# flashlight/wav2letter

Hardware: AMD Instinct MI355X
Metric: utterances/sec (higher is better)
Workload: dtype f32

## Files before the change

### include/fl_compat/flashlight.h

```cpp
#pragma once
#include <stdint.h>
#include <cstdio>
#include <initializer_list>

#include <functional>
#include <memory>
#include <stdexcept>
#include <string>
#include <type_traits>
#include <unordered_map>
#include <utility>
#include <vector>

#define FL_COMPAT_API __attribute__((visibility("default")))

namespace af {
typedef long long dim_t;

class FL_COMPAT_API dim4 {
 public:
  dim_t dims[4];
  dim4(dim_t d0 = 1, dim_t d1 = 1, dim_t d2 = 1, dim_t d3 = 1) : dims{d0, d1, d2, d3} {}
  dim_t elements() const { return dims[0] * dims[1] * dims[2] * dims[3]; }
  dim_t ndims() const {
// ... 386 lines not shown

 private:
  std::shared_ptr<fl::Sequential> net_;
  std::shared_ptr<void> state_;
  void* h_ = nullptr;
  int slots_ = 0, maxChunk_ = 0, maxOut_ = 0, nFeat_ = 0, nLabel_ = 0;
  bool mixed_ = false;
};

class FL_COMPAT_API SequenceCriterion : public fl::Container {
 public:
  std::vector<Variable> forward(const std::vector<Variable>& inputs) override = 0;
  virtual af::array viterbiPath(const af::array& input, const af::array& inputSize = af::array()) = 0;
  virtual af::array viterbiPathWithTarget(const af::array& input, const af::array& target,
                                          const af::array& inputSizes = af::array(), const af::array& targetSizes = af::array()) = 0;
  std::string prettyString() const override = 0;
};

struct FlatView { float* ptr; size_t floats; };
FL_COMPAT_API FlatView flatParameters(const std::shared_ptr<fl::Module>& network);
FL_COMPAT_API FlatView flatGradients(const std::shared_ptr<fl::Module>& network);
FL_COMPAT_API void setMixedPrecision(const std::shared_ptr<fl::Module>& network, bool on);
FL_COMPAT_API void setMixedPrecisionConvolutions(const std::shared_ptr<fl::Module>& network, bool on);
FL_COMPAT_API uint32_t networkStep(const std::shared_ptr<fl::Module>& network);
FL_COMPAT_API void setNetworkStep(const std::shared_ptr<fl::Module>& network, uint32_t step);

class NGramLM;
class Lexicon;

struct BeamSearchOptions {
  int beamSize = 64;
  int beamSizeToken = 64;
  float beamThreshold = 1.0f / 0.0f;
  bool logAdd = false;
  int normalize = -1;
  int nbest = 1;
  int maxLen = 0;
  const NGramLM* lm = nullptr;
  float lmWeight = 0.f;
  af::array classScore;
  float eosScore = 0.f;
  const Lexicon* lexicon = nullptr;
  float wordScore = 0.f;
  int maxWords = 0;
  bool wide = false;
};
// ... 84 lines not shown
```

### include/w2l_hip.h

```cpp
#ifndef W2L_HIP_H_
#define W2L_HIP_H_

#include <stddef.h>
#include <stdint.h>

#ifdef __cplusplus
extern "C" {
#endif

typedef void* w2l_stream_t;

typedef enum {
  W2L_OK = 0,
  W2L_EINVAL = 1,
  W2L_EHIP = 2,
  W2L_EUNSUPPORTED = 3
} w2l_status;

typedef enum {
  W2L_SCALE_NONE = 0,
  W2L_SCALE_INPUT_SZ = 1,
  W2L_SCALE_INPUT_SZ_SQRT = 2,
  W2L_SCALE_TARGET_SZ = 3,
  W2L_SCALE_TARGET_SZ_SQRT = 4
// ... 359 lines not shown
int w2l_trainer_param_info(void* h, int i, char* name, int nameCap, size_t* numel, size_t* offset);
int w2l_trainer_init_params(void* h, float* h_params, uint64_t seed);
int w2l_trainer_import_param(void* h, int i, const float* h_ref, float* h_params);
int w2l_trainer_export_param(void* h, int i, const float* h_arena, float* h_ref);
int w2l_trainer_plan(void* h, int B, int T, int L, size_t* arenaFloats, size_t* critWsBytes, int* Tout);
int w2l_trainer_bind(void* h, float* params, float* grads, float* momentum, float* arena, void* critWs);
int w2l_trainer_forward(void* h, const float* x, int train, const float** emission, void* stream);
int w2l_trainer_forward_backward(void* h, const float* x, const int* target, float** lossDev,
                                 void* stream);
int w2l_trainer_backward(void* handle, const float* dEmission, void* stream);
int w2l_trainer_update(void* h, float lr, float lrcrit, float momentum, float maxGradNorm,
                       float totalBatch, int clampCrit, void* stream);
int w2l_trainer_skipped_updates(void* h, uint64_t* count, void* stream);
int w2l_trainer_set_optimizer(void* h, int netKind, int critKind);
int w2l_trainer_set_input_sizes(void* h, const float* inputSizesDev);
int w2l_trainer_bind_state2(void* h, float* state2);
int w2l_trainer_viterbi(void* h, const float* emission, int* path, void* stream);
int w2l_trainer_evaluate(void* h, const float* x, const int* target, float** lossDev, int** pathDev, void* stream);
size_t w2l_trainer_eval_bytes(void* h);
int w2l_trainer_bind_eval(void* h, void* mem, size_t bytes);
int w2l_trainer_set_step(void* h, uint32_t step);
int w2l_trainer_set_mixed_precision(void* h, int on);
int w2l_trainer_set_mixed_precision_convs(void* h, int on);
int w2l_trainer_set_dropout(void* h, double pDropout, double pLayerDrop);
int w2l_trainer_grad_norm(void* h, double* norm, void* stream);
int w2l_trainer_set_linseg(void* h, uint32_t updates);
int w2l_trainer_set_grad_buckets(void* h, int n, const size_t* offsets);
int w2l_trainer_wait_bucket(void* h, int k, void* stream);
int w2l_profile_enable(int on);
int w2l_profile_report(int* launches, double* totalMs, double* totalFlops);
int w2l_profile_report_kind(int kind, int* launches, double* totalMs, double* totalWork);
int w2l_profile_launches(int kind, int maxRows, double* ms, double* work, int* dims);
int w2l_arch_check(const char* archText, int nFeat, int nLabel, int* numLayers);
int w2l_flags_check(const char* flagsText, int* numFlags);

int w2l_stream_create(const char* archText, int nFeat, int nLabel, int slots, int maxChunk, void** session);
int w2l_stream_create_for_trainer(void* trainer, int slots, int maxChunk, void** session);
void w2l_stream_destroy(void* session);
int w2l_stream_query(const char* archText, int nFeat, int nLabel, int slots, int maxChunk, int* maxOut, size_t* stateBytes);
int w2l_stream_max_out(void* session);
size_t w2l_stream_state_bytes(void* session);
size_t w2l_stream_param_floats(void* session);
int w2l_stream_num_time_layers(void* session);
int w2l_stream_bind(void* session, const float* params, void* state, size_t stateBytes);
int w2l_stream_counts(void* session, const int* n, const int* start, const int* finish, int* nOut);
int w2l_stream_slot_state(void* session, int slot, int* active, int* carry, int carryCap);
// ... 50 lines not shown
```

### wav2letter_amd/csrc/gemm.hip

```cpp
#include <atomic>
#include <cstdlib>
#include <map>
#include <mutex>
#include <utility>

#include "gemm.hpp"
#include "gemm_glds.hpp"
#include "gemm_t160.hpp"
#include "gemm_bf16.hpp"
#include "gemm_bf16g.hpp"

namespace w2l {

GemmProf& gemm_prof() {
  static GemmProf p;
  return p;
}

float* sk_scratch(hipStream_t s, size_t bytes) {
  static std::mutex mu;
  static std::map<std::pair<int, hipStream_t>, std::pair<float*, size_t>> cache;
  int dev = 0;
  if (hipGetDevice(&dev) != hipSuccess) return nullptr;
  std::lock_guard<std::mutex> lk(mu);
  auto& e = cache[{dev, s}];
  if (e.second < bytes) {
    if (e.first) (void)hipFree(e.first);
    e.first = nullptr;
    e.second = 0;
    void* p = nullptr;
    if (hipMalloc(&p, bytes) != hipSuccess) return nullptr;
    e.first = (float*)p;
    e.second = bytes;
  }
  return e.first;
}

static bool glds_enabled() {
  const char* e = tune_env("W2L_GEMM_GLDS");
  return !(e && e[0] == '0');
}

static inline bool glds_ok(const float* p, int ld, int extent) {
  return (((uintptr_t)p) & 15) == 0 && ld % 4 == 0 && extent % 4 == 0 && extent >= 4;
}
static inline bool glds_ok_relaxed(const float* p, int extent) {
  return (((uintptr_t)p) & 3) == 0 && extent >= 4;
}

unsigned* sk_counters(hipStream_t s) {
  static std::mutex mu;
  static std::map<std::pair<int, hipStream_t>, unsigned*> cache;
  int dev = 0;
  if (hipGetDevice(&dev) != hipSuccess) return nullptr;
  std::lock_guard<std::mutex> lk(mu);
  unsigned*& e = cache[{dev, s}];
  if (!e) {
    void* p = nullptr;
    if (hipMalloc(&p, 1024 * sizeof(unsigned)) != hipSuccess) return nullptr;
    if (hipMemset(p, 0, 1024 * sizeof(unsigned)) != hipSuccess) { (void)hipFree(p); return nullptr; }
    e = (unsigned*)p;
  }
  return e;
}

template <class AOp>
static int dispatch_b(const AOp& a, const float* B, int ldb, int b_kcontig, const GemmOut& o, int epi, hipStream_t s) {
  if (b_kcontig) {
    int v = pick_vec(B, ldb, o.K);
    if (v == 4) return launch128(a, PlainOp<true, 4>{B, ldb, o.N, o.K}, o, epi, s);
    if (v == 2) return launch128(a, PlainOp<true, 2>{B, ldb, o.N, o.K}, o, epi, s);
    return launch128(a, PlainOp<true, 1>{B, ldb, o.N, o.K}, o, epi, s);
  }
  int v = pick_vec(B, ldb, o.N);
  if (v == 4) return launch128(a, PlainOp<false, 4>{B, ldb, o.N, o.K}, o, epi, s);
  if (v == 2) return launch128(a, PlainOp<false, 2>{B, ldb, o.N, o.K}, o, epi, s);
  return launch128(a, PlainOp<false, 1>{B, ldb, o.N, o.K}, o, epi, s);
}

static std::atomic<int> g_matmul_bf16{0};

static int gemm_bf16(const float* A, int lda, int a_kcontig, const float* B, int ldb, int b_kcontig, const GemmOut& o, int epi,
                     hipStream_t s) {
  const bool va = pick_vec(A, lda, a_kcontig ? o.K : o.M) == 4, vb = pick_vec(B, ldb, b_kcontig ? o.K : o.N) == 4;
  if (a_kcontig) {
    const BfOp<true> a{A, lda, o.M, o.K, va};
// ... 248 lines not shown
```

### wav2letter_amd/csrc/host/fl_compat.cpp

```cpp
#include <dlfcn.h>
#include <time.h>

#include <algorithm>
#include <cmath>
#include <cstring>
#include <sstream>
#include <unordered_map>
#include <unordered_set>

#include "../../../include/fl_compat/flashlight.h"
#include "../../../include/fl_compat/lexicon.h"
#include "../../../include/fl_compat/lm.h"
#include "w2l_host.hpp"

namespace {

hipStream_t g_stream = nullptr;
bool g_streamUser = false;

hipStream_t S() {
  if (!g_stream) w2l::hipCheck(hipStreamCreateWithFlags(&g_stream, hipStreamNonBlocking), "fl_compat stream");
  return g_stream;
}

// ... 1030 lines not shown
hipEvent_t arenaBucketEvent(void* net, size_t k) { return ((pkg::speech::PlannedNet*)net)->bucketEvents_.at(k); }
void arenaInstallBuckets(void* net, std::vector<size_t> offs) { ((pkg::speech::PlannedNet*)net)->installBuckets(std::move(offs)); }
}
namespace pkg {
namespace speech {

namespace {
PlannedNet* plannedOf(fl::Module* m) {
  if (auto* p = dynamic_cast<PlannedNet*>(m)) return p;
  if (auto* s = dynamic_cast<fl::Sequential*>(m)) return dynamic_cast<PlannedNet*>(s->planned().get());
  return nullptr;
}
}

FlatView flatParameters(const std::shared_ptr<fl::Module>& network) {
  auto* p = plannedOf(network.get());
  return p ? FlatView{p->paramPtr(), p->impl().paramFloats()} : FlatView{nullptr, 0};
}
void setMixedPrecision(const std::shared_ptr<fl::Module>& network, bool on) {
  if (auto* p = plannedOf(network.get())) p->mixed_ = on;
}
void setMixedPrecisionConvolutions(const std::shared_ptr<fl::Module>& network, bool on) {
  if (auto* p = plannedOf(network.get())) p->setMixedConvs(on);
}
uint32_t networkStep(const std::shared_ptr<fl::Module>& network) {
  auto* p = plannedOf(network.get());
  return p ? p->step() : 0;
}
void setNetworkStep(const std::shared_ptr<fl::Module>& network, uint32_t step) {
  if (auto* p = plannedOf(network.get())) p->setStep(step);
}
FlatView flatGradients(const std::shared_ptr<fl::Module>& network) {
  auto* p = plannedOf(network.get());
  return p ? FlatView{p->gradPtr(), p->impl().paramFloats()} : FlatView{nullptr, 0};
}

namespace {

struct CritState {
  std::shared_ptr<w2l::SequenceCriterion> impl;
  std::shared_ptr<void> ws;
  size_t wsBytes = 0;
  void* workspace(int B, int T, int N, int L) {
    const size_t need = impl->workspaceBytes(B, T, N, L) + 256;
    if (need > wsBytes) { ws = devAlloc(need); wsBytes = need; }
    return ws.get();
// ... 832 lines not shown
```

### wav2letter_amd/csrc/host/net.cpp

```cpp
#include <algorithm>
#include <cmath>
#include <cstring>
#include <sstream>

#include "w2l_host.hpp"

namespace w2l {

std::string Act::str() const {
  std::ostringstream os;
  os << "(";
  for (int i = 0; i < 4; ++i) {
    os << (i ? "," : "");
    if (d[i].f.size() == 1 && d[i].f[0].kind == F_TIME) os << "T";
    else if (d[i].f.size() == 1 && d[i].f[0].kind == F_BATCH) os << "B";
    else os << d[i].size();
  }
  os << ") phys[" << B << "][" << T << "][" << F << "]";
  return os.str();
}

static constexpr int kSymT = 1000003, kSymB = 1000033;

Act actInput(int B, int T, int nFeat) {
  Act a;
// ... 309 lines not shown
    return true;
  }
  void backwardData(Ctx& c, float* arena, const BfImage& dyImg, float* dx, const float* mask, float maskScale, const float* addend,
                    int accumulate) const {
    w2l_gemm_epilogue e{};
    e.mask = mask; e.maskScale = maskScale; e.addend = addend; e.accumulate = accumulate;
    w2lCheck(w2l_gemm_bf16(M, in, out, dyImg.r(arena), dyImg.colsP, w.r(arena), w.colsP, dx, in, nullptr, 0,
                           (mask || addend || accumulate) ? &e : nullptr, c.stream), "bf16 linear bwd data");
  }
  void backwardWeight(Ctx& c, float* arena, const BfImage& xImg, const BfImage& dyImg, float* dw, bool withBias = false) const {
    w2lCheck(w2l_gemm_bf16(in + (withBias ? 1 : 0), out, M, xImg.t(arena), xImg.rowsP, dyImg.t(arena), dyImg.rowsP, dw, out, nullptr, 0,
                           nullptr, c.stream), "bf16 linear bwd weight");
  }
  bool biasRides(const BfImage& xImg, const float* dw, const float* db) const {
    return xImg.onesRow && db == dw + (size_t)in * out;
  }
};

struct FeedForward {
  const char* who = "";
  const P *w1 = nullptr, *b1 = nullptr, *w2 = nullptr, *b2 = nullptr;
  bool joinInLin2 = true;
  bool biasWithWeight = false;
  int M = 0, in = 0, hidden = 0;
  size_t uOff = 0, duOff = 0;
  BfLinear bl1, bl2;
  BfImage uImg, duImg;
  bool uOnlyImages = false;
  void plan(Planner& pl, const char* who_, int M_, int in_, int hidden_, const P& w1_, const P& b1_, const P& w2_, const P& b2_) {
    who = who_; M = M_; in = in_; hidden = hidden_; w1 = &w1_; b1 = &b1_; w2 = &w2_; b2 = &b2_;
    uOff = pl.alloc((size_t)M * hidden); duOff = pl.alloc((size_t)M * hidden);
    bl1.plan(pl, M, in, hidden); bl2.plan(pl, M, hidden, in);
    uImg.plan(pl, M, hidden, true); duImg.plan(pl, M, hidden);
  }
  std::string tag(const char* what) const { return std::string(who) + " " + what; }
  void check(int st, const char* what) const { if (st != W2L_OK) w2lCheck(st, tag(what).c_str()); }
  bool lin2BiasRides(Ctx& cx) const { return bl2.biasRides(uImg, w2->g(cx), b2->g(cx)); }
  bool forward(Ctx& cx, float* ar, const float* x, const BfImage& xImg, float* out, double p, uint32_t stream) {
    float* u = ar + uOff;
    if (cx.bf16) {
      uOnlyImages = bl1.forwardImages(cx, ar, xImg, b1->w(cx), uImg, 1, p, cx.seed, stream);
      if (!uOnlyImages) {
        bl1.forward(cx, ar, xImg, b1->w(cx), u, 1, p, cx.seed, stream);
        uImg.convert(cx, ar, u, tag("u images").c_str());
      }
      bl2.forwardAdd(cx, ar, uImg, b2->w(cx), x, out, p, cx.seed, stream + 1);
      return true;
    }
    if (p > 0) check(w2l_linear_forward_dropout(M, in, hidden, x, w1->w(cx), b1->w(cx), u, 1, p, cx.seed, stream, cx.stream), "lin1+do");
    else check(w2l_linear_forward(M, in, hidden, x, w1->w(cx), b1->w(cx), u, 1, cx.stream), "lin1");
    if (joinInLin2) check(w2l_linear_forward_dropout_add(M, hidden, in, u, w2->w(cx), b2->w(cx), x, out, 0, p, cx.seed, stream + 1, cx.stream), "lin2+do+res");
    else check(w2l_linear_forward(M, hidden, in, u, w2->w(cx), b2->w(cx), out, 0, cx.stream), "lin2");
    return joinInLin2;
  }
  void weightGrad(Ctx& cx, float* ar, const BfLinear& bl, const float* a, const BfImage& aImg, const float* g, const BfImage& gImg, const P& w, const P& b,
                  bool rides) const {
    if (cx.bf16) bl.backwardWeight(cx, ar, aImg, gImg, w.g(cx), rides);
    else if (rides) check(w2l_linear_backward_weight_bias(M, bl.in, bl.out, a, g, w.g(cx), b.g(cx), cx.stream), "bwd w + b");
    else check(w2l_linear_backward_weight(M, bl.in, bl.out, a, g, w.g(cx), cx.stream), "bwd w");
    if (!rides) check(w2l_colsum(g, b.g(cx), (size_t)M, bl.out, cx.stream), "bwd b");
  }
  void backward(Ctx& cx, float* ar, const float* x, const BfImage& xImg, const float* dy, const BfImage& dyImg, const float* addend, float* dx, double p) {
    const bool mixed = cx.bf16;
    const bool rides2 = mixed ? lin2BiasRides(cx) : biasWithWeight, rides1 = mixed ? bl1.biasRides(xImg, w1->g(cx), b1->g(cx)) : biasWithWeight;
    const float sc = (float)(1.0 / (1.0 - p));
    float *u = ar + uOff, *du = ar + duOff;
    weightGrad(cx, ar, bl2, u, uImg, dy, dyImg, *w2, *b2, rides2);
    if (!mixed) {
      check(w2l_linear_backward_data(M, hidden, in, dy, w2->w(cx), du, 0, u, sc, cx.stream), "lin2 bwd x");
    } else if (!(uOnlyImages && bl2.backwardDataImages(cx, ar, dyImg, rides1 ? nullptr : du, &duImg, uImg, sc))) {
      if (uOnlyImages) throw std::runtime_error(tag("u was kept as images only, but the image-writing backward-data product refused"));
      bl2.backwardData(cx, ar, dyImg, du, u, sc, nullptr, 0);
      duImg.convert(cx, ar, du, tag("du images").c_str());
    }
    weightGrad(cx, ar, bl1, x, xImg, du, duImg, *w1, *b1, rides1);
    if (mixed) bl1.backwardData(cx, ar, duImg, dx, nullptr, 1.f, addend, 0);
    else check(w2l_linear_backward_data_add(M, in, hidden, du, w1->w(cx), addend, dx, cx.stream), "lin1 bwd x");
  }
};

constexpr size_t kLnImageElems = (size_t)1 << 22;
static bool lnForward(Ctx& cx, float* ar, int groups, size_t inner, float* a, const float* x, float* r, float* y, const float* gb, double p,
                      uint32_t seed, uint32_t stream, double* stats, float* mr, const BfImage* img, const char* what) {
// ... 126 lines not shown
      return;
    }
    if (wide(c)) {
      w2lCheck(w2l_conv_bf16_prepare(&d, wt, bfp(arena, wideImgFOff), bfp(arena, wideImgBOff), c.stream), "wide conv images");
      w2lCheck(w2l_conv_bf16_forward(&d, x, bfp(arena, wideImgFOff), hasBias ? b.w(c) : nullptr, y, fuseRelu ? 1 : 0, c.convScratch, c.stream),
               "wide conv fwd bf16");
      return;
    }
    w2lCheck(w2l_conv_forward(&d, x, wt, hasBias ? b.w(c) : nullptr, y, fuseRelu ? 1 : 0, c.stream), "conv fwd");
  }
  bool wide(const Ctx& c) const { return c.bf16 && wideImgElems && c.convScratch; }
  void backward(Ctx& c, float* arena, const float* dy, float*& dx, bool needDx) override {
    float* dym = const_cast<float*>(dy);
    if (fuseRelu) w2lCheck(w2l_mask_backward(dy, arena + yOff, dym, nOut, 1.f, c.stream), "conv relu bwd");
    float* dwt = wn.on ? arena + wn.dwOff : w.g(c);
    const bool bf = c.bf16 && convImgElems;
    const bool wd = wide(c);
    if (wd) {
      w2lCheck(w2l_conv_bf16_backward_filter_bias(&d, xSaved, dym, dwt, hasBias ? b.g(c) : nullptr, c.convScratch, c.stream),
               "wide conv bwd filter + bias bf16");
    } else if (bf) {
      w2lCheck(w2l_tds_conv_bf16_backward_filter_bias(&d, xSaved, dym, dwt, hasBias ? b.g(c) : nullptr, c.stream), "conv bwd filter + bias bf16");
    } else {
      w2lCheck(w2l_conv_backward_filter(&d, xSaved, dym, dwt, hasBias ? b.g(c) : nullptr, c.stream), "conv bwd filter");
    }
    const float* wt = wn.on ? arena + wn.wOff : w.w(c);
    if (needDx) {
      dx = arena + dxOff;
      if (wd) {
        w2lCheck(w2l_conv_bf16_backward_data(&d, dym, bfp(arena, wideImgBOff), nullptr, kh > 1 ? arena + dxeOff : dx, c.convScratch, c.stream),
                 "wide conv bwd data bf16");
        if (kh > 1) w2lCheck(w2l_hexpand_backward(arena + dxeOff, dx, (size_t)d.B * d.T, d.H, cin, kh, padH, c.stream), "conv H fold");
      } else if (bf && kh > 1) {
        w2lCheck(w2l_tds_conv_bf16_backward_data(&d, dym, bfp(arena, convImgBOff), nullptr, arena + dxeOff, c.stream), "conv bwd data bf16");
        w2lCheck(w2l_hexpand_backward(arena + dxeOff, dx, (size_t)d.B * d.T, d.H, cin, kh, padH, c.stream), "conv H fold");
      } else if (bf) {
        w2lCheck(w2l_tds_conv_bf16_backward_data(&d, dym, bfp(arena, convImgBOff), nullptr, dx, c.stream), "conv bwd data bf16");
      } else if (kh > 1) {
        w2lCheck(w2l_conv_backward_data(&d, dym, wt, arena + dxeOff, 0, c.stream), "conv bwd data");
        w2lCheck(w2l_hexpand_backward(arena + dxeOff, dx, (size_t)d.B * d.T, d.H, cin, kh, padH, c.stream), "conv H fold");
      } else {
        w2lCheck(w2l_conv_backward_data(&d, dym, wt, dx, 0, c.stream), "conv bwd data");
      }
    }
    if (wn.on)
      w2lCheck(w2l_weightnorm_backward(wn.v.w(c), wn.g.w(c), arena + wn.normOff, dwt, wn.v.g(c), wn.g.g(c),
                                       arena + wn.dotOff, wn.K, wn.N, c.stream), "wn bwd");
// ... 101 lines not shown
        xImg.convert(c, arena, x, "linear input images");
      }
      if (!c.weightsReady) bl.convertWeight(c, arena, wt);
      bl.forward(c, arena, xSeen, hasBias ? b.w(c) : nullptr, y, fuseRelu ? 1 : 0, 0.0, 0, 0);
      return;
    }
    w2lCheck(w2l_linear_forward(M, in, out, x, wt, hasBias ? b.w(c) : nullptr, y, fuseRelu ? 1 : 0, c.stream), "linear fwd");
  }
  void backward(Ctx& c, float* arena, const float* dy, float*& dx, bool needDx) override {
    float* dym = const_cast<float*>(dy);
    if (fuseRelu) w2lCheck(w2l_mask_backward(dy, arena + yOff, dym, (size_t)M * out, 1.f, c.stream), "linear relu bwd");
    float* dwt = wn.on ? arena + wn.dwOff : w.g(c);
    const float* wt = wn.on ? arena + wn.wOff : w.w(c);
    if (c.bf16) {
      dyImg.convert(c, arena, dym, "linear output-gradient images");
      const bool rides = hasBias && bl.biasRides(xSeen, dwt, b.g(c));
      bl.backwardWeight(c, arena, xSeen, dyImg, dwt, rides);
      if (hasBias && !rides) w2lCheck(w2l_colsum(dym, b.g(c), (size_t)M, out, c.stream), "linear bwd b");
      if (needDx) {
        dx = arena + dxOff;
        bl.backwardData(c, arena, dyImg, dx, nullptr, 1.f, nullptr, 0);
      }
    } else {
    w2lCheck(w2l_linear_backward_weight_bias(M, in, out, xSaved, dym, dwt, hasBias ? b.g(c) : nullptr, c.stream), "linear bwd w + b");
    if (needDx) {
      dx = arena + dxOff;
      w2lCheck(w2l_linear_backward_data(M, in, out, dym, wt, dx, 0, nullptr, 1.f, c.stream), "linear bwd x");
    }
    }
    if (wn.on)
      w2lCheck(w2l_weightnorm_backward(wn.v.w(c), wn.g.w(c), arena + wn.normOff, dwt, wn.v.g(c), wn.g.g(c),
                                       arena + wn.dotOff, wn.K, wn.N, c.stream), "wn bwd");
  }
};

class LayerNormLayer : public Layer {
 public:
  bool streamGeom(StreamGeom& g, std::string& why) const override {
    std::vector<int> ax = axes;
    std::sort(ax.begin(), ax.end());
    if (ax != std::vector<int>{1, 2}) { why = "LayerNorm over the time axis needs the whole utterance"; return false; }
    g = StreamGeom();
    return true;
  }
  std::vector<int> axes;
  P gb;
  int groups = 0;
// ... 109 lines not shown
  }
  Act plan(const Act& in, Planner& pl) override {
    int H;
    requireConvLayout(in, c, "TDSBlock", H);
    if (H != h) throw std::invalid_argument("TDSBlock: expected H=" + std::to_string(h) + ", input " + in.str());
    int pL, pR;
    if (rPad < 0) { pL = pR = samePad(in.T, kw, 1); }
    else { if (rPad > kw - 1) throw std::invalid_argument("TDSBlock: invalid right padding"); pR = rPad; pL = kw - 1 - rPad; }
    if (streamMode_) pL = pR = 0;
    d = {in.B, in.T, h, c, c, kw, 1, pL, pR};
    const int To = w2l_conv_out_len(in.T, kw, 1, pL, pR);
    if (!streamMode_ && To != in.T) throw std::invalid_argument("TDSBlock: conv must preserve T (odd kw)");
    if (To <= 0) throw std::invalid_argument("TDSBlock: input too short: " + in.str());
    B = in.B; T = To; M = B * T; n = (size_t)M * in.F;
    groups = lnTime ? B : B * T;
    inner = n / groups;
    if (inner % 4 && !streamMode_) throw std::invalid_argument("TDSBlock: LayerNorm size must be a multiple of 4");
    aOff = pl.alloc(n); r1Off = pl.alloc(n); y1Off = pl.alloc(n); vOff = pl.alloc(n); outOff = pl.alloc(n);
    st1Off = pl.alloc(2 * w2l_layernorm_scratch_doubles(groups, inner)); mr1Off = pl.alloc(2 * (size_t)groups);
    st2Off = pl.alloc(2 * w2l_layernorm_scratch_doubles(groups, inner)); mr2Off = pl.alloc(2 * (size_t)groups);
    dsOff = pl.alloc(n); dy1Off = pl.alloc(n); dr1Off = pl.alloc(n); daOff = pl.alloc(n); dxOff = pl.alloc(n);
    ff.joinInLin2 = l2 % 32 == 0;
    ff.biasWithWeight = true;
    ff.plan(pl, "tds", M, l, l2, w1, b1, w2, b2);
    y1Img.plan(pl, M, l, true); dvImg.plan(pl, M, l);
    convImgElems = h % 16 == 0 ? w2l_tds_conv_bf16_image_elems(&d) : 0;
    if (convImgElems) { convImgFOff = pl.allocBf16(convImgElems); convImgBOff = pl.allocBf16(convImgElems); }
    Act o = in;
    o.T = To;
    return o;
  }
  void forward(Ctx& cx, float* ar, const float* x, float*& y) override {
    hipStream_t s = cx.stream;
    const double pd = cx.train ? p : 0.0;
    xSaved = x;
    const float* xr = x;
    if (streamMode_) {
      if (!cx.streamRes) throw std::logic_error("TDSBlock in stream mode without its residual frames");
      xr = cx.streamRes;
    }
    float *a = ar + aOff, *r1 = ar + r1Off, *y1 = ar + y1Off, *v = ar + vOff, *out = ar + outOff;
    if (cx.bf16 && convImgElems) {
      if (!cx.weightsReady) w2lCheck(w2l_tds_conv_bf16_prepare(&d, wc.w(cx), bfp(ar, convImgFOff), bfp(ar, convImgBOff), s), "tds conv images");
      w2lCheck(w2l_tds_conv_bf16_forward(&d, x, bfp(ar, convImgFOff), bc.w(cx), a, 1, s), "tds conv bf16");
    } else {
      w2lCheck(w2l_conv_forward(&d, x, wc.w(cx), bc.w(cx), a, 1, s), "tds conv");
// ... 5 lines not shown
      const int first = y1Images ? 1 : 0, count = (cx.weightsReady ? 1 : 3) - first;
      if (count > 0) w2lCheck(w2l_bf16_convert_multi(count, wd + first, s), "tds y1 + weight images");
      if (!y1Images) y1Img.ensureOnes(cx, ar);
    }
    const bool joined = ff.forward(cx, ar, y1, y1Img, v, pd, rngStream + 1);
    float* r2 = (inner & 3) ? r1 : v;
    w2lCheck(w2l_residual_layernorm_forward(groups, inner, v, joined ? nullptr : y1, r2, out, gb2.w(cx), 1e-5f, joined ? 0.0 : pd,
                                            joined ? 0 : cx.seed, joined ? 0 : rngStream + 2, (double*)(ar + st2Off), ar + mr2Off, s), "tds ln2");
    y = out;
  }
  void backward(Ctx& cx, float* ar, const float* dy, float*& dx, bool needDx) override {
    hipStream_t s = cx.stream;
    const double pd = cx.train ? p : 0.0;
    const float sc = (float)(1.0 / (1.0 - pd));
    float *a = ar + aOff, *y1 = ar + y1Off, *v = ar + vOff;
    float *ds = ar + dsOff, *dy1 = ar + dy1Off, *dr1 = ar + dr1Off, *da = ar + daOff;
    const bool rides2 = cx.bf16 && ff.lin2BiasRides(cx);
    const bool maskInConvert = pd > 0 && rides2;
    const bool dvImages = lnBackward(cx, ar, groups, inner, v, dy, gb2.w(cx), ar + mr2Off, ds, gb2.g(cx), nullptr, nullptr, 1.f,
                                     (double*)(ar + st2Off), cx.bf16 && (pd == 0 || maskInConvert) ? &dvImg : nullptr, pd, cx.seed,
                                     rngStream + 2, "tds ln2 bwd");
    const float* dv = ds;
    if (pd > 0 && !maskInConvert) {
      w2lCheck(w2l_dropout_copy(dy1, ds, n, pd, cx.seed, rngStream + 2, s), "tds do2 bwd");
      dv = dy1;
    }
    if (cx.bf16 && !dvImages) {
      if (maskInConvert) dvImg.convertDropout(cx, ar, ds, pd, cx.seed, rngStream + 2, "tds dv images (masked)");
      else dvImg.convert(cx, ar, dv, "tds dv images");
    }
    ff.backward(cx, ar, y1, y1Img, dv, dvImg, ds, dy1, pd);
    w2lCheck(w2l_layernorm_backward(groups, inner, ar + r1Off, dy1, gb1.w(cx), ar + mr1Off, dr1, gb1.g(cx), a, da, sc,
                                    (double*)(ar + st1Off), s), "tds ln1 bwd");
    if (cx.bf16 && convImgElems) {
      w2lCheck(w2l_tds_conv_bf16_backward_filter_bias(&d, xSaved, da, wc.g(cx), bc.g(cx), s), "tds conv bwd filter + bias bf16");
      if (needDx) {
        dx = ar + dxOff;
        w2lCheck(w2l_tds_conv_bf16_backward_data(&d, da, bfp(ar, convImgBOff), dr1, dx, s), "tds conv bwd data bf16");
      }
      return;
    }
    w2lCheck(w2l_conv_backward_filter(&d, xSaved, da, wc.g(cx), bc.g(cx), s), "tds conv bwd filter");
    if (needDx) {
      dx = ar + dxOff;
      w2lCheck(w2l_conv_backward_data_add(&d, da, wc.w(cx), dr1, dx, s), "tds conv bwd data");
    }
  }
};

class PoolTimeLayer : public Layer {
 public:
  int w = 1, stride = 1;
  int B = 0, T = 0, To = 0, F = 0;
  size_t yOff = 0, dxOff = 0;
  const float* xSaved = nullptr;
  std::string name() const override { return "Pool2D"; }
  Act plan(const Act& in, Planner& pl) override {
    if (!isKind(in.d[0], F_TIME) || !isKind(in.d[3], F_BATCH))
      throw std::invalid_argument("Pool2D: input must be (T, H, C, B), got " + in.str());
    if (in.T < w) throw std::invalid_argument("Pool2D: fewer frames than the window");
    B = in.B; T = in.T; F = in.F;
    To = (T - w) / stride + 1;
    Act o = in;
    o.T = To;
    yOff = pl.alloc((size_t)B * To * F);
// ... 412 lines not shown
  convScratchOff_ = convScratchElems_ ? pl.allocBf16(convScratchElems_) : 0;
  return pl.used();
}

const float* Sequential::forward(Ctx& c, float* arena, const float* xRef) {
  float* x = arena + inOff_;
  w2lCheck(w2l_transpose(xRef, x, in_.B, in_.F, in_.T, c.stream), "input transpose");
  const float* cur = x;
  c.imgOf = nullptr;
  c.convScratch = convScratchElems_ ? bfp(arena, convScratchOff_) : nullptr;
  for (size_t i = 0; i < layers_.size(); ++i) {
    float* y = nullptr;
    const float* noteBefore = c.imgOf;
    layers_[i]->forward(c, arena, cur, y);
    if (c.imgOf == noteBefore && !layers_[i]->passesInputThrough(c)) c.imgOf = nullptr;
    if (c.imgOf != y) c.imgOf = nullptr;
    ys_[i] = y;
    cur = y;
  }
  c.imgOf = nullptr;
  return cur;
}

void Sequential::backward(Ctx& c, float* arena, const float* dOut) {
  const float* dy = dOut;
  c.convScratch = convScratchElems_ ? bfp(arena, convScratchOff_) : nullptr;
  size_t firstParam = 0;
  for (size_t i = 0; i < layers_.size(); ++i) {
    const std::string nm = layers_[i]->name();
    if (nm != "View" && nm != "Reorder" && nm != "SpecAugment" && nm != "Dropout" && nm != "ReLU") { firstParam = i; break; }
  }
  size_t nb = bOff_.size();
  for (size_t ii = layers_.size(); ii-- > 0;) {
    float* dx = nullptr;
    bool needDx = ii > firstParam;
    layers_[ii]->backward(c, arena, dy, dx, needDx);
    for (; nb > 0 && bOff_[nb - 1] >= layerLo_[ii]; --nb) hipCheck(hipEventRecord(bEv_[nb - 1], c.stream), "bucket event");
    if (!needDx) break;
    dy = dx;
  }
  for (; nb > 0; --nb) hipCheck(hipEventRecord(bEv_[nb - 1], c.stream), "bucket event");
}

static inline uint64_t splitmix(uint64_t& s) {
  uint64_t z = (s += 0x9E3779B97F4A7C15ull);
  z = (z ^ (z >> 30)) * 0xBF58476D1CE4E5B9ull;
  z = (z ^ (z >> 27)) * 0x94D049BB133111EBull;
  return z ^ (z >> 31);
}

void Sequential::importParam(size_t i, const float* ref, float* host) const {
  const ParamInfo& p = params_[i];
  float* dst = host + p.offset;
  if (p.kind == 1) {
    for (int co = 0; co < p.cout; ++co)
      for (int ci = 0; ci < p.cin; ++ci)
        for (int dh = 0; dh < p.kh; ++dh)
          for (int k = 0; k < p.kw; ++k)
            dst[(((size_t)k * p.kh + dh) * p.cin + ci) * p.cout + co] = ref[(((size_t)co * p.cin + ci) * p.kh + dh) * p.kw + k];
  } else if (p.kind == 2 && !p.rowPerm.empty()) {
    for (int r = 0; r < p.cin; ++r) std::memcpy(dst + (size_t)r * p.cout, ref + (size_t)p.rowPerm[r] * p.cout, sizeof(float) * p.cout);
  } else if (p.kind == 5) {
    for (int r = 0; r < p.cin; ++r)
      for (int c = 0; c < p.cout; ++c) dst[(size_t)r * p.cout + c] = ref[(size_t)c * p.cin + r];
// ... 205 lines not shown
```

### wav2letter_amd/csrc/host/trainer.cpp

```cpp
#include <cmath>
#include <cstring>
#include <map>
#include <mutex>
#include <vector>

#include <algorithm>

#include "w2l_host.hpp"

namespace w2l {

struct Trainer {
  std::shared_ptr<Sequential> net;
  std::shared_ptr<SequenceCriterion> crit;
  int nFeat = 0, nLabel = 0;
  std::string critName;
  std::string archText;
  int B = 0, T = 0, L = 0, Tout = 0;
  size_t netFloats = 0, critFloats = 0, arenaFloats = 0, critWsBytes = 0;
  float *params = nullptr, *grads = nullptr, *mom = nullptr, *arena = nullptr;
  void* critWs = nullptr;
  float *loss = nullptr, *gradLoss = nullptr, *dEm = nullptr;
  double* sumsq = nullptr;
  float* batchSlot = nullptr;
// ... 352 lines not shown
      hipCheck(hipStreamSynchronize((hipStream_t)stream), "skipped");
    }
    *count = (uint64_t)s;
  });
}

W2L_API int w2l_trainer_set_optimizer(void* h, int netKind, int critKind) {
  if (!h || netKind < 0 || netKind > 2 || critKind < 0 || critKind > 2) return W2L_EINVAL;
  ((Trainer*)h)->netOptim = netKind; ((Trainer*)h)->critOptim = critKind;
  return W2L_OK;
}
W2L_API int w2l_trainer_set_input_sizes(void* h, const float* inputSizesDev) {
  if (!h) return W2L_EINVAL;
  ((Trainer*)h)->inputSizes = inputSizesDev;
  return W2L_OK;
}
W2L_API int w2l_trainer_bind_state2(void* h, float* state2) {
  if (!h) return W2L_EINVAL;
  ((Trainer*)h)->state2 = state2;
  return W2L_OK;
}
W2L_API int w2l_trainer_set_mixed_precision(void* h, int on) { ((Trainer*)h)->mixedPrecision = on != 0; return W2L_OK; }

W2L_API int w2l_trainer_set_mixed_precision_convs(void* h, int on) {
  if (!h) return W2L_EINVAL;
  Trainer* t = (Trainer*)h;
  if (t->net->mixedPrecisionConvs() == (on != 0)) return W2L_OK;
  t->net->setMixedPrecisionConvs(on != 0);
  t->arenaFloats = 0;
  t->params = t->grads = t->mom = t->arena = nullptr;
  t->critWs = nullptr;
  return W2L_OK;
}

W2L_API int w2l_trainer_set_dropout(void* h, double pDropout, double pLayerDrop) {
  if (!h || !(pDropout < 1.0) || !(pLayerDrop < 1.0)) return W2L_EINVAL;
  ((Trainer*)h)->net->setTransformerDropout(pDropout, pLayerDrop);
  return W2L_OK;
}

W2L_API int w2l_trainer_set_step(void* h, uint32_t step) { ((Trainer*)h)->step = step; return W2L_OK; }

W2L_API int w2l_arch_check(const char* archText, int nFeat, int nLabel, int* numLayers) {
  TRY(nullptr, { auto v = parseArch(archText, nFeat, nLabel); if (numLayers) *numLayers = (int)v.size(); });
}
W2L_API int w2l_flags_check(const char* flagsText, int* numFlags) {
// ... 3 lines not shown
```

### wav2letter_amd/csrc/host/w2l_host.hpp

```cpp
#pragma once
#include <hip/hip_runtime.h>
#include <stdint.h>

#include <memory>
#include <stdexcept>
#include <string>
#include <vector>

#include "../../../include/w2l_hip.h"

namespace w2l {

struct LayerSpec {
  std::string tok;
  std::vector<std::string> args;
  std::string line;
  int lineNo = 0;
  std::shared_ptr<LayerSpec> child;
};
std::vector<LayerSpec> parseArch(const std::string& text, int64_t nFeat, int64_t nLabel);
std::string readFile(const std::string& path);

enum FKind { F_FEAT = 0, F_TIME = 1, F_BATCH = 2 };
struct Factor {
// ... 24 lines not shown
  std::vector<int> rowPerm;
  double initBound = 0;
  float initConst = 0;
  int kw = 0, kh = 1, cin = 0, cout = 0;
};

struct Ctx {
  hipStream_t stream = nullptr;
  bool train = true;
  uint32_t seed = 0;
  float* params = nullptr;
  float* grads = nullptr;
  const float* inputSizes = nullptr;
  int inputT = 0;
  const float* inputSizeFull = nullptr;
  bool bf16 = false;
  const float* imgOf = nullptr;
  size_t imgRowsOff = 0, imgTransOff = 0;
  int imgRows = 0, imgCols = 0;
  uint16_t* convScratch = nullptr;
  const float* streamRes = nullptr;
  bool smallM = false;
  bool weightsReady = false;
};

struct StreamGeom {
  bool timeExtent = false;
  int kw = 1, stride = 1, padL = 0, padR = 0;
  int resShift = -1;
};

class Planner {
 public:
  size_t alloc(size_t floats) { size_t o = used_; used_ += (floats + 63) / 64 * 64; return o; }
  size_t allocBf16(size_t elements) { return alloc((elements + 1) / 2); }
  size_t used() const { return used_; }
  bool bf16Convs = false;
  void wantConvScratch(size_t bf16Elements) { if (bf16Elements > convScratch_) convScratch_ = bf16Elements; }
  size_t convScratch() const { return convScratch_; }
 private:
  size_t used_ = 0;
  size_t convScratch_ = 0;
};

class Layer {
 public:
  virtual ~Layer() {}
  virtual std::string name() const = 0;
  virtual void registerParams(std::vector<ParamInfo>& table) { (void)table; }
  virtual Act plan(const Act& in, Planner& pl) = 0;
  virtual void forward(Ctx& c, float* arena, const float* x, float*& y) = 0;
  virtual void backward(Ctx& c, float* arena, const float* dy, float*& dx, bool needDx) = 0;
  virtual bool passesInputThrough(const Ctx& c) const { (void)c; return false; }
  virtual void setTransformerDropout(double pDropout, double pLayerDrop) { (void)pDropout; (void)pLayerDrop; }
  int rngStream = 0;
  virtual bool streamGeom(StreamGeom& g, std::string& why) const { (void)g; why = "the layer needs the whole utterance"; return false; }
  void setStreamMode(bool on) { streamMode_ = on; }
  std::string archLine;
 protected:
  bool streamMode_ = false;
};

class Sequential {
 public:
  void add(std::shared_ptr<Layer> l) { layers_.push_back(std::move(l)); }
  size_t size() const { return layers_.size(); }
  Layer& at(size_t i) { return *layers_[i]; }
  std::string prettyString() const;

  void finalize();
  void setTransformerDropout(double pDropout, double pLayerDrop) { for (auto& l : layers_) l->setTransformerDropout(pDropout, pLayerDrop); }
  void setMixedPrecisionConvs(bool on) { bf16Convs_ = on; }
  bool mixedPrecisionConvs() const { return bf16Convs_; }
  const std::vector<ParamInfo>& params() const { return params_; }
  size_t paramFloats() const { return paramFloats_; }

  size_t plan(int B, int T, int nFeat);
  const Act& outAct() const { return out_; }
  const Act& inAct() const { return in_; }

  const float* forward(Ctx& c, float* arena, const float* xRef);
  void backward(Ctx& c, float* arena, const float* dOut);

  void setGradBuckets(std::vector<size_t> offsets, std::vector<hipEvent_t> events) { bOff_ = std::move(offsets); bEv_ = std::move(events); }

  void initParams(float* hostParams, uint64_t seed) const;
  void importParam(size_t i, const float* ref, float* hostParams) const;
  void exportParam(size_t i, const float* hostArena, float* ref) const;

 private:
  std::vector<std::shared_ptr<Layer>> layers_;
  std::vector<ParamInfo> params_;
  size_t paramFloats_ = 0;
  Act in_, out_;
  size_t inOff_ = 0;
  bool bf16Convs_ = false;
  size_t convScratchOff_ = 0, convScratchElems_ = 0;
  std::vector<size_t> dOff_;
  std::vector<Act> acts_;
  std::vector<float*> ys_;
  std::vector<size_t> layerLo_;
  std::vector<size_t> bOff_;
  std::vector<hipEvent_t> bEv_;
};

std::shared_ptr<Sequential> buildSequentialModule(const std::string& archfile, int64_t nFeatures, int64_t nClasses);
std::shared_ptr<Sequential> buildSequentialFromText(const std::string& archText, int64_t nFeatures, int64_t nClasses, bool dryPlan = true);
void requireEmissionLayout(const Act& out);

class SequenceCriterion {
 public:
  virtual ~SequenceCriterion() {}
  virtual std::string prettyString() const = 0;
  virtual size_t paramFloats() const { return 0; }
  virtual void initParams(float* host) const { (void)host; }
  virtual size_t workspaceBytes(int B, int T, int N, int L) const = 0;
  virtual void forward(Ctx& c, int B, int T, int N, int L, const float* emission, const int* target,
                       float* loss, void* ws, float* critParams) = 0;
  virtual void backward(Ctx& c, int B, int T, int N, int L, const float* emission, const int* target,
                        const float* gradLoss, float* dEmission, void* ws, float* critParams,
                        float* critGrads) = 0;
  virtual void viterbiPath(Ctx& c, int B, int T, int N, const float* emission, int* path, void* ws,
                           float* critParams) = 0;
  virtual size_t scoreWorkspaceBytes(int B, int T, int N, int L) const { return workspaceBytes(B, T, N, L); }
  virtual void score(Ctx& c, int B, int T, int N, int L, const float* emission, const int* target, float* loss, int* path,
                     void* ws, float* critParams) {
    forward(c, B, T, N, L, emission, target, loss, ws, critParams);
// ... 43 lines not shown
```

### wav2letter_amd/trainer.py

```python
import ctypes as C

import numpy as np
import torch

from . import _lib
from .criterion import CriterionScaleMode

_sigs_done = set()


def _lib_tr():
    L = _lib.lib()
    if id(L) not in _sigs_done:
        vp, i, sz, f, d, u32, u64 = C.c_void_p, C.c_int, C.c_size_t, C.c_float, C.c_double, C.c_uint32, C.c_uint64
        L.w2l_host_last_error.restype = C.c_char_p
        L.w2l_trainer_create.restype = vp
        L.w2l_trainer_create.argtypes = [C.c_char_p, i, i, C.c_char_p, i, d]
        L.w2l_trainer_destroy.argtypes = [vp]
        L.w2l_trainer_describe.restype = C.c_char_p
        L.w2l_trainer_describe.argtypes = [vp]
        for n in ("w2l_trainer_param_floats", "w2l_trainer_net_param_floats", "w2l_trainer_grad_floats"):
            getattr(L, n).restype = sz
            getattr(L, n).argtypes = [vp]
        L.w2l_trainer_num_params.argtypes = [vp]
        L.w2l_trainer_param_info.argtypes = [vp, i, C.c_char_p, i, C.POINTER(sz), C.POINTER(sz)]
        L.w2l_trainer_init_params.argtypes = [vp, vp, u64]
        L.w2l_trainer_import_param.argtypes = [vp, i, vp, vp]
        L.w2l_trainer_export_param.argtypes = [vp, i, vp, vp]
        L.w2l_trainer_plan.argtypes = [vp, i, i, i, C.POINTER(sz), C.POINTER(sz), C.POINTER(i)]
        L.w2l_trainer_bind.argtypes = [vp, vp, vp, vp, vp, vp]
        L.w2l_trainer_forward.argtypes = [vp, vp, i, C.POINTER(vp), vp]
        L.w2l_trainer_forward_backward.argtypes = [vp, vp, vp, C.POINTER(vp), vp]
        L.w2l_trainer_backward.argtypes = [vp, vp, vp]
        L.w2l_trainer_update.argtypes = [vp, f, f, f, f, f, i, vp]
        L.w2l_trainer_viterbi.argtypes = [vp, vp, vp, vp]
        L.w2l_trainer_evaluate.argtypes = [vp, vp, vp, C.POINTER(vp), C.POINTER(vp), vp]
        L.w2l_trainer_eval_bytes.restype = sz
        L.w2l_trainer_eval_bytes.argtypes = [vp]
        L.w2l_trainer_bind_eval.argtypes = [vp, vp, sz]
        L.w2l_trainer_set_step.argtypes = [vp, u32]
        L.w2l_trainer_set_mixed_precision.argtypes = [vp, i]
        L.w2l_trainer_set_mixed_precision_convs.argtypes = [vp, i]
        L.w2l_trainer_set_optimizer.argtypes = [vp, i, i]
        L.w2l_trainer_set_dropout.argtypes = [vp, d, d]
        L.w2l_trainer_bind_state2.argtypes = [vp, vp]
        L.w2l_trainer_set_input_sizes.argtypes = [vp, vp]
        L.w2l_trainer_set_linseg.argtypes = [vp, u32]
        L.w2l_trainer_grad_norm.argtypes = [vp, C.POINTER(C.c_double), vp]
        L.w2l_trainer_skipped_updates.argtypes = [vp, C.POINTER(u64), vp]
        L.w2l_trainer_set_grad_buckets.argtypes = [vp, i, C.POINTER(sz)]
        L.w2l_trainer_wait_bucket.argtypes = [vp, i, vp]
        L.w2l_arch_check.argtypes = [C.c_char_p, i, i, C.POINTER(i)]
        L.w2l_flags_check.argtypes = [C.c_char_p, C.POINTER(i)]
        _sigs_done.add(id(L))
    return L


def _check(st, what):
    if st != 0:
        msg = _lib_tr().w2l_host_last_error().decode()
        if st == _lib.W2L_EINVAL:
            raise _lib.W2LInvalidArgument(f"{what}: {msg}")
        raise _lib.W2LError(f"{what}: {msg}")


# ... 216 lines not shown
        _check(self.L.w2l_trainer_viterbi(self.h, emission.data_ptr(), path.data_ptr(), self._stream()), "viterbi")
        return path

    def grad_norm(self):
        n = C.c_double(0.0)
        _check(self.L.w2l_trainer_grad_norm(self.h, C.byref(n), self._stream()), "grad_norm")
        return n.value

    def skipped_updates(self):
        n = C.c_uint64(0)
        _check(self.L.w2l_trainer_skipped_updates(self.h, C.byref(n), self._stream()), "skipped_updates")
        return n.value

    def set_mixed_precision(self, on=True, convs=False):
        _check(self.L.w2l_trainer_set_mixed_precision(self.h, int(bool(on))), "mixed precision")
        self._mixed = bool(on)
        if bool(convs) != self._mixed_convs:
            _check(self.L.w2l_trainer_set_mixed_precision_convs(self.h, int(bool(convs))), "mixed precision convolutions")
            self._mixed_convs = bool(convs)
            self._eval_plans.clear()
            if self.B:
                self.plan(self.B, self.T, self.Lt)

    def set_optimizer(self, netoptim="sgd", critoptim="sgd"):
        kinds = {"sgd": 0, "adagrad": 1, "adadelta": 2}
        _check(self.L.w2l_trainer_set_optimizer(self.h, kinds[netoptim], kinds[critoptim]), "set_optimizer")
        self._optim = (netoptim, critoptim)
        self._bind_state2()

    def set_input_sizes(self, sizes):
        if sizes is not None:
            if not (torch.is_tensor(sizes) and sizes.dtype == torch.float32 and sizes.is_cuda and sizes.is_contiguous()
                    and sizes.numel() == self.B):
                raise ValueError("input sizes: contiguous float32 CUDA tensor of B elements")
        self._input_sizes = sizes
        _check(self.L.w2l_trainer_set_input_sizes(self.h, sizes.data_ptr() if sizes is not None else None), "set_input_sizes")

    def set_step(self, step):
        self.L.w2l_trainer_set_step(self.h, step)

    def set_linseg(self, updates):
        _check(self.L.w2l_trainer_set_linseg(self.h, int(updates)), "linseg")

    def set_grad_buckets(self, offsets):
        arr = (C.c_size_t * len(offsets))(*offsets)
        _check(self.L.w2l_trainer_set_grad_buckets(self.h, len(offsets), arr), "set_grad_buckets")
# ... 5 lines not shown
```

Baseline: 329.3.

## Run fp32 weight-gradient kernels on a side stream overlapping data-gradient backward

Adds a secondary non-blocking HIP stream per network. During fp32 training backward, weight and bias gradient GEMMs and convolution filter-gradient kernels fork onto it via events, so they can run concurrently with the data-gradient chain. Bucket events are recorded on the side stream and a join event resynchronizes at the end of backward. Scratch buffers are warmed for both streams. The change adds event overhead per layer and a possible race on shared scratch, and it is disabled for bf16 and when profiling.

```diff
diff --git a/include/fl_compat/flashlight.h b/include/fl_compat/flashlight.h
--- a/include/fl_compat/flashlight.h
+++ b/include/fl_compat/flashlight.h
@@ -432,6 +432,7 @@
 FL_COMPAT_API FlatView flatGradients(const std::shared_ptr<fl::Module>& network);
 FL_COMPAT_API void setMixedPrecision(const std::shared_ptr<fl::Module>& network, bool on);
 FL_COMPAT_API void setMixedPrecisionConvolutions(const std::shared_ptr<fl::Module>& network, bool on);
+FL_COMPAT_API void setWeightGradStream(const std::shared_ptr<fl::Module>& network, bool on);
 FL_COMPAT_API uint32_t networkStep(const std::shared_ptr<fl::Module>& network);
 FL_COMPAT_API void setNetworkStep(const std::shared_ptr<fl::Module>& network, uint32_t step);
 
diff --git a/include/w2l_hip.h b/include/w2l_hip.h
--- a/include/w2l_hip.h
+++ b/include/w2l_hip.h
@@ -405,6 +405,7 @@
 int w2l_trainer_set_step(void* h, uint32_t step);
 int w2l_trainer_set_mixed_precision(void* h, int on);
 int w2l_trainer_set_mixed_precision_convs(void* h, int on);
+int w2l_trainer_set_weight_grad_stream(void* h, int on);
 int w2l_trainer_set_dropout(void* h, double pDropout, double pLayerDrop);
 int w2l_trainer_grad_norm(void* h, double* norm, void* stream);
 int w2l_trainer_set_linseg(void* h, uint32_t updates);
diff --git a/wav2letter_amd/csrc/gemm.hip b/wav2letter_amd/csrc/gemm.hip
--- a/wav2letter_amd/csrc/gemm.hip
+++ b/wav2letter_amd/csrc/gemm.hip
@@ -16,6 +16,7 @@
   static GemmProf p;
   return p;
 }
+bool profileEnabled() { return gemm_prof().on; }
 
 float* sk_scratch(hipStream_t s, size_t bytes) {
   static std::mutex mu;
@@ -62,6 +63,11 @@
     e = (unsigned*)p;
   }
   return e;
+}
+
+void warmStreamScratch(hipStream_t s) {
+  (void)sk_scratch(s, kSkScratchBytes);
+  (void)sk_counters(s);
 }
 
 template <class AOp>
diff --git a/wav2letter_amd/csrc/host/fl_compat.cpp b/wav2letter_amd/csrc/host/fl_compat.cpp
--- a/wav2letter_amd/csrc/host/fl_compat.cpp
+++ b/wav2letter_amd/csrc/host/fl_compat.cpp
@@ -1076,6 +1076,9 @@
 }
 void setMixedPrecisionConvolutions(const std::shared_ptr<fl::Module>& network, bool on) {
   if (auto* p = plannedOf(network.get())) p->setMixedConvs(on);
+}
+void setWeightGradStream(const std::shared_ptr<fl::Module>& network, bool on) {
+  if (auto* p = plannedOf(network.get())) p->impl().setWeightGradStream(on);
 }
 uint32_t networkStep(const std::shared_ptr<fl::Module>& network) {
   auto* p = plannedOf(network.get());
diff --git a/wav2letter_amd/csrc/host/net.cpp b/wav2letter_amd/csrc/host/net.cpp
--- a/wav2letter_amd/csrc/host/net.cpp
+++ b/wav2letter_amd/csrc/host/net.cpp
@@ -1,6 +1,7 @@
 #include <algorithm>
 #include <cmath>
 #include <cstring>
+#include <mutex>
 #include <sstream>
 
 #include "w2l_host.hpp"
@@ -356,6 +357,7 @@
   const P *w1 = nullptr, *b1 = nullptr, *w2 = nullptr, *b2 = nullptr;
   bool joinInLin2 = true;
   bool biasWithWeight = false;
+  bool offChain = false;
   int M = 0, in = 0, hidden = 0;
   size_t uOff = 0, duOff = 0;
   BfLinear bl1, bl2;
@@ -389,10 +391,11 @@
   }
   void weightGrad(Ctx& cx, float* ar, const BfLinear& bl, const float* a, const BfImage& aImg, const float* g, const BfImage& gImg, const P& w, const P& b,
                   bool rides) const {
+    hipStream_t s = (offChain && !cx.bf16) ? cx.forkWeightGrad() : cx.stream;
     if (cx.bf16) bl.backwardWeight(cx, ar, aImg, gImg, w.g(cx), rides);
-    else if (rides) check(w2l_linear_backward_weight_bias(M, bl.in, bl.out, a, g, w.g(cx), b.g(cx), cx.stream), "bwd w + b");
-    else check(w2l_linear_backward_weight(M, bl.in, bl.out, a, g, w.g(cx), cx.stream), "bwd w");
-    if (!rides) check(w2l_colsum(g, b.g(cx), (size_t)M, bl.out, cx.stream), "bwd b");
+    else if (rides) check(w2l_linear_backward_weight_bias(M, bl.in, bl.out, a, g, w.g(cx), b.g(cx), s), "bwd w + b");
+    else check(w2l_linear_backward_weight(M, bl.in, bl.out, a, g, w.g(cx), s), "bwd w");
+    if (!rides) check(w2l_colsum(g, b.g(cx), (size_t)M, bl.out, s), "bwd b");
   }
   void backward(Ctx& cx, float* ar, const float* x, const BfImage& xImg, const float* dy, const BfImage& dyImg, const float* addend, float* dx, double p) {
     const bool mixed = cx.bf16;
@@ -565,7 +568,7 @@
     } else if (bf) {
       w2lCheck(w2l_tds_conv_bf16_backward_filter_bias(&d, xSaved, dym, dwt, hasBias ? b.g(c) : nullptr, c.stream), "conv bwd filter + bias bf16");
     } else {
-      w2lCheck(w2l_conv_backward_filter(&d, xSaved, dym, dwt, hasBias ? b.g(c) : nullptr, c.stream), "conv bwd filter");
+      w2lCheck(w2l_conv_backward_filter(&d, xSaved, dym, dwt, hasBias ? b.g(c) : nullptr, wn.on ? c.stream : c.forkWeightGrad()), "conv bwd filter");
     }
     const float* wt = wn.on ? arena + wn.wOff : w.w(c);
     if (needDx) {
@@ -713,7 +716,8 @@
         bl.backwardData(c, arena, dyImg, dx, nullptr, 1.f, nullptr, 0);
       }
     } else {
-    w2lCheck(w2l_linear_backward_weight_bias(M, in, out, xSaved, dym, dwt, hasBias ? b.g(c) : nullptr, c.stream), "linear bwd w + b");
+    w2lCheck(w2l_linear_backward_weight_bias(M, in, out, xSaved, dym, dwt, hasBias ? b.g(c) : nullptr, wn.on ? c.stream : c.forkWeightGrad()),
+             "linear bwd w + b");
     if (needDx) {
       dx = arena + dxOff;
       w2lCheck(w2l_linear_backward_data(M, in, out, dym, wt, dx, 0, nullptr, 1.f, c.stream), "linear bwd x");
@@ -869,6 +873,7 @@
     dsOff = pl.alloc(n); dy1Off = pl.alloc(n); dr1Off = pl.alloc(n); daOff = pl.alloc(n); dxOff = pl.alloc(n);
     ff.joinInLin2 = l2 % 32 == 0;
     ff.biasWithWeight = true;
+    ff.offChain = true;
     ff.plan(pl, "tds", M, l, l2, w1, b1, w2, b2);
     y1Img.plan(pl, M, l, true); dvImg.plan(pl, M, l);
     convImgElems = h % 16 == 0 ? w2l_tds_conv_bf16_image_elems(&d) : 0;
@@ -920,8 +925,9 @@
                                      rngStream + 2, "tds ln2 bwd");
     const float* dv = ds;
     if (pd > 0 && !maskInConvert) {
-      w2lCheck(w2l_dropout_copy(dy1, ds, n, pd, cx.seed, rngStream + 2, s), "tds do2 bwd");
-      dv = dy1;
+      float* masked = cx.bf16 ? dy1 : v;
+      w2lCheck(w2l_dropout_copy(masked, ds, n, pd, cx.seed, rngStream + 2, s), "tds do2 bwd");
+      dv = masked;
     }
     if (cx.bf16 && !dvImages) {
       if (maskInConvert) dvImg.convertDropout(cx, ar, ds, pd, cx.seed, rngStream + 2, "tds dv images (masked)");
@@ -938,7 +944,7 @@
       }
       return;
     }
-    w2lCheck(w2l_conv_backward_filter(&d, xSaved, da, wc.g(cx), bc.g(cx), s), "tds conv bwd filter");
+    w2lCheck(w2l_conv_backward_filter(&d, xSaved, da, wc.g(cx), bc.g(cx), cx.forkWeightGrad()), "tds conv bwd filter");
     if (needDx) {
       dx = ar + dxOff;
       w2lCheck(w2l_conv_backward_data_add(&d, da, wc.w(cx), dr1, dx, s), "tds conv bwd data");
@@ -1397,9 +1403,77 @@
   return cur;
 }
 
+hipStream_t Ctx::forkWeightGrad() {
+  if (!wgStream) return stream;
+  hipCheck(hipEventRecord(wgFork, stream), "weight-gradient fork");
+  hipCheck(hipStreamWaitEvent(wgStream, wgFork, 0), "weight-gradient fork");
+  return wgStream;
+}
+
+namespace {
+std::mutex g_wgMu;
+std::vector<std::pair<int, hipStream_t>> g_wgFree;
+}
+
+void Sequential::wgRelease() {
+  if (wgStream_) {
+    std::lock_guard<std::mutex> lk(g_wgMu);
+    g_wgFree.emplace_back(wgDev_, wgStream_);
+  }
+  if (wgFork_) (void)hipEventDestroy(wgFork_);
+  if (wgJoin_) (void)hipEventDestroy(wgJoin_);
+  wgStream_ = nullptr; wgFork_ = wgJoin_ = nullptr; wgDev_ = -1;
+}
+Sequential::~Sequential() { wgRelease(); }
+
+struct Sequential::WgScope {
+  Sequential& n;
+  Ctx& c;
+  bool joined = true;
+  WgScope(Sequential& n_, Ctx& c_) : n(n_), c(c_) {
+    c.wgStream = nullptr; c.wgFork = nullptr;
+    if (!n.wgOn_ || !c.train || c.bf16 || profileEnabled()) return;
+    int dev = 0;
+    hipCheck(hipGetDevice(&dev), "weight-gradient stream");
+    if (n.wgStream_ && dev != n.wgDev_) n.wgRelease();
+    if (!n.wgStream_) {
+      {
+        std::lock_guard<std::mutex> lk(g_wgMu);
+        for (size_t i = 0; i < g_wgFree.size(); ++i)
+          if (g_wgFree[i].first == dev) { n.wgStream_ = g_wgFree[i].second; g_wgFree.erase(g_wgFree.begin() + i); break; }
+      }
+      n.wgDev_ = dev;
+      try {
+        if (!n.wgStream_) hipCheck(hipStreamCreateWithFlags(&n.wgStream_, hipStreamNonBlocking), "weight-gradient stream");
+        hipCheck(hipEventCreateWithFlags(&n.wgFork_, hipEventDisableTiming), "weight-gradient fork event");
+        hipCheck(hipEventCreateWithFlags(&n.wgJoin_, hipEventDisableTiming), "weight-gradient join event");
+      } catch (...) {
+        n.wgRelease();
+        throw;
+      }
+      warmStreamScratch(n.wgStream_);
+      warmStreamScratch(c.stream);
+    }
+    c.wgStream = n.wgStream_; c.wgFork = n.wgFork_;
+    joined = false;
+  }
+  hipError_t joinNoThrow() {
+    if (joined) return hipSuccess;
+    joined = true;
+    hipError_t e = hipEventRecord(n.wgJoin_, n.wgStream_);
+    if (e == hipSuccess) e = hipStreamWaitEvent(c.stream, n.wgJoin_, 0);
+    c.wgStream = nullptr; c.wgFork = nullptr;
+    return e;
+  }
+  void join() { hipCheck(joinNoThrow(), "weight-gradient join"); }
+  ~WgScope() { (void)joinNoThrow(); }
+  void recordBucket(hipEvent_t ev) { hipCheck(hipEventRecord(ev, c.forkWeightGrad()), "bucket event"); }
+};
+
 void Sequential::backward(Ctx& c, float* arena, const float* dOut) {
   const float* dy = dOut;
   c.convScratch = convScratchElems_ ? bfp(arena, convScratchOff_) : nullptr;
+  WgScope wg(*this, c);
   size_t firstParam = 0;
   for (size_t i = 0; i < layers_.size(); ++i) {
     const std::string nm = layers_[i]->name();
@@ -1410,11 +1484,12 @@
     float* dx = nullptr;
     bool needDx = ii > firstParam;
     layers_[ii]->backward(c, arena, dy, dx, needDx);
-    for (; nb > 0 && bOff_[nb - 1] >= layerLo_[ii]; --nb) hipCheck(hipEventRecord(bEv_[nb - 1], c.stream), "bucket event");
+    for (; nb > 0 && bOff_[nb - 1] >= layerLo_[ii]; --nb) wg.recordBucket(bEv_[nb - 1]);
     if (!needDx) break;
     dy = dx;
   }
-  for (; nb > 0; --nb) hipCheck(hipEventRecord(bEv_[nb - 1], c.stream), "bucket event");
+  for (; nb > 0; --nb) wg.recordBucket(bEv_[nb - 1]);
+  wg.join();
 }
 
 static inline uint64_t splitmix(uint64_t& s) {
diff --git a/wav2letter_amd/csrc/host/trainer.cpp b/wav2letter_amd/csrc/host/trainer.cpp
--- a/wav2letter_amd/csrc/host/trainer.cpp
+++ b/wav2letter_amd/csrc/host/trainer.cpp
@@ -398,6 +398,12 @@
 }
 W2L_API int w2l_trainer_set_mixed_precision(void* h, int on) { ((Trainer*)h)->mixedPrecision = on != 0; return W2L_OK; }
 
+W2L_API int w2l_trainer_set_weight_grad_stream(void* h, int on) {
+  if (!h) return W2L_EINVAL;
+  ((Trainer*)h)->net->setWeightGradStream(on != 0);
+  return W2L_OK;
+}
+
 W2L_API int w2l_trainer_set_mixed_precision_convs(void* h, int on) {
   if (!h) return W2L_EINVAL;
   Trainer* t = (Trainer*)h;
diff --git a/wav2letter_amd/csrc/host/w2l_host.hpp b/wav2letter_amd/csrc/host/w2l_host.hpp
--- a/wav2letter_amd/csrc/host/w2l_host.hpp
+++ b/wav2letter_amd/csrc/host/w2l_host.hpp
@@ -70,6 +70,9 @@
   const float* streamRes = nullptr;
   bool smallM = false;
   bool weightsReady = false;
+  hipStream_t wgStream = nullptr;
+  hipEvent_t wgFork = nullptr;
+  hipStream_t forkWeightGrad();
 };
 
 struct StreamGeom {
@@ -111,6 +114,10 @@
 
 class Sequential {
  public:
+  Sequential() {}
+  ~Sequential();
+  Sequential(const Sequential&) = delete;
+  Sequential& operator=(const Sequential&) = delete;
   void add(std::shared_ptr<Layer> l) { layers_.push_back(std::move(l)); }
   size_t size() const { return layers_.size(); }
   Layer& at(size_t i) { return *layers_[i]; }
@@ -131,6 +138,9 @@
   void backward(Ctx& c, float* arena, const float* dOut);
 
   void setGradBuckets(std::vector<size_t> offsets, std::vector<hipEvent_t> events) { bOff_ = std::move(offsets); bEv_ = std::move(events); }
+
+  void setWeightGradStream(bool on) { wgOn_ = on; }
+  bool weightGradStream() const { return wgOn_; }
 
   void initParams(float* hostParams, uint64_t seed) const;
   void importParam(size_t i, const float* ref, float* hostParams) const;
@@ -150,7 +160,15 @@
   std::vector<size_t> layerLo_;
   std::vector<size_t> bOff_;
   std::vector<hipEvent_t> bEv_;
-};
+  struct WgScope;
+  bool wgOn_ = true;
+  int wgDev_ = -1;
+  hipStream_t wgStream_ = nullptr;
+  hipEvent_t wgFork_ = nullptr, wgJoin_ = nullptr;
+  void wgRelease();
+};
+bool profileEnabled();
+void warmStreamScratch(hipStream_t s);
 
 std::shared_ptr<Sequential> buildSequentialModule(const std::string& archfile, int64_t nFeatures, int64_t nClasses);
 std::shared_ptr<Sequential> buildSequentialFromText(const std::string& archText, int64_t nFeatures, int64_t nClasses, bool dryPlan = true);
diff --git a/wav2letter_amd/trainer.py b/wav2letter_amd/trainer.py
--- a/wav2letter_amd/trainer.py
+++ b/wav2letter_amd/trainer.py
@@ -41,6 +41,7 @@
         L.w2l_trainer_set_step.argtypes = [vp, u32]
         L.w2l_trainer_set_mixed_precision.argtypes = [vp, i]
         L.w2l_trainer_set_mixed_precision_convs.argtypes = [vp, i]
+        L.w2l_trainer_set_weight_grad_stream.argtypes = [vp, i]
         L.w2l_trainer_set_optimizer.argtypes = [vp, i, i]
         L.w2l_trainer_set_dropout.argtypes = [vp, d, d]
         L.w2l_trainer_bind_state2.argtypes = [vp, vp]
@@ -303,6 +304,9 @@
             if self.B:
                 self.plan(self.B, self.T, self.Lt)
 
+    def set_weight_grad_stream(self, on=True):
+        _check(self.L.w2l_trainer_set_weight_grad_stream(self.h, int(bool(on))), "weight-gradient stream")
+
     def set_optimizer(self, netoptim="sgd", critoptim="sgd"):
         kinds = {"sgd": 0, "adagrad": 1, "adadelta": 2}
         _check(self.L.w2l_trainer_set_optimizer(self.h, kinds[netoptim], kinds[critoptim]), "set_optimizer")
```

New measurement: 338.3 (median of 6 runs). +2.7%, better.
